# HJakeCunningham/ASVGP

Hardware: AMD Instinct MI355X
Metric: Mpoints/s per ELBO+grad step, N=10M 1D Matern-3/2 M=2048 (higher is better)
Workload: dtype f64

## Files before the change

### asvgp_amd/csrc/bcr_mfma.hpp

```cpp
#pragma once
#include "bcr.hpp"
#include "prior_plan.hpp"

namespace asvgp {

constexpr int BM_THREADS = 1024;
constexpr int BM_B = 4;
constexpr int BM_GAT = 0, BM_GBT = 16, BM_DINV = 32, BM_SD = 48, BM_CAT = 64, BM_CBT = 80, BM_W = 96, BM_DG = 100, BM_REC = 104;

__host__ __device__ inline size_t bcr_mfma_ws_doubles(long nb) { return (size_t)nb * BM_REC + 64; }
__host__ __device__ inline size_t bcr_mfma_lds_doubles(long nb) {
  return (size_t)((nb + 1) / 2 + 1) * 32 + (size_t)nb * 4 + 96 + (size_t)(BM_THREADS / 64) * 4 * 40 + (size_t)(nb / 8 + 2) * 52;
}

__device__ __forceinline__ double bm_mfma(double a, double b, double c) { return __builtin_amdgcn_mfma_f64_4x4x4f64(a, b, c, 0, 0, 0); }

__device__ __forceinline__ double bm_chol_linv(const double (&d)[10], int hi, int lo, double& dprod, int& badj) {
  double l00, i0, l10, l20, l30, l11, i1, l21, l31, l22, i2, l32, l33, i3;
  Num<double>::sqrt_inv(d[0], l00, i0);
  badj = !(d[0] > 0.0) ? 1 : 0;
  l10 = d[1] * i0; l20 = d[3] * i0; l30 = d[6] * i0;
  double s = fma(-l10, l10, d[2]);
  badj = (!(s > 0.0) && !badj) ? 2 : badj;
  Num<double>::sqrt_inv(s, l11, i1);
  l21 = fma(-l20, l10, d[4]) * i1;
  l31 = fma(-l30, l10, d[7]) * i1;
  s = fma(-l21, l21, fma(-l20, l20, d[5]));
  badj = (!(s > 0.0) && !badj) ? 3 : badj;
  Num<double>::sqrt_inv(s, l22, i2);
  l32 = fma(-l31, l21, fma(-l30, l20, d[8])) * i2;
  s = fma(-l32, l32, fma(-l31, l31, fma(-l30, l30, d[9])));
  badj = (!(s > 0.0) && !badj) ? 4 : badj;
  Num<double>::sqrt_inv(s, l33, i3);
  dprod = (l00 * l11) * (l22 * l33);
  const double z0 = (lo == 0) ? i0 : 0.0;
  const double z1 = fma(-l10, z0, (lo == 1) ? 1.0 : 0.0) * i1;
  const double z2 = fma(-l21, z1, fma(-l20, z0, (lo == 2) ? 1.0 : 0.0)) * i2;
  const double z3 = fma(-l32, z2, fma(-l31, z1, fma(-l30, z0, (lo == 3) ? 1.0 : 0.0))) * i3;
  return hi == 0 ? z0 : (hi == 1 ? z1 : (hi == 2 ? z2 : z3));
}

template <typename Src> __device__ __forceinline__ auto bm_src_load(const Src& A, int dd, long col, long M, int) -> decltype(A.load_dc(dd, col, M)) {
  return A.load_dc(dd, col, M);
}
template <typename Src> __device__ __forceinline__ double bm_src_load(const Src& A, int dd, long col, long M, long) {
  return A.load((long)dd * M + col, true);
}
struct BmLog {
  double m; int e;
  __device__ __forceinline__ void mul(double p) {
    m *= p;
    const int hi = __double2hiint(m);
    e += ((hi >> 20) & 0x7ff) - 1023;
    m = __hiloint2double((hi & 0x800fffff) | 0x3ff00000, __double2loint(m));
  }
};

__device__ __forceinline__ unsigned long long bm_wave_xor(unsigned long long x) {
#pragma unroll
  for (int off = 32; off > 0; off >>= 1) x ^= (unsigned long long)__shfl_xor((long long)x, off, 64);
  return x;
}
__device__ __forceinline__ void bm_msg_send(double* box, int n, double v, unsigned long long tag, int lane) {
  unsigned long long* b = reinterpret_cast<unsigned long long*>(box);
  const unsigned long long w = lane < n ? (unsigned long long)__double_as_longlong(v) : 0ull;
  const unsigned long long x = bm_wave_xor(w) ^ tag;
  if (lane < n) __hip_atomic_store(b + lane, w, __ATOMIC_RELAXED, __HIP_MEMORY_SCOPE_AGENT);
  if (lane == n) __hip_atomic_store(b + n, x, __ATOMIC_RELAXED, __HIP_MEMORY_SCOPE_AGENT);
}
__device__ __forceinline__ bool bm_msg_recv(const double* box, int n, double& v, unsigned long long tag, int lane, long spin_limit) {
  const unsigned long long* b = reinterpret_cast<const unsigned long long*>(box);
  for (long spins = 0; spins <= spin_limit; ++spins) {
    const unsigned long long w = lane <= n ? __hip_atomic_load(b + lane, __ATOMIC_RELAXED, __HIP_MEMORY_SCOPE_AGENT) : 0ull;
    const unsigned long long x = bm_wave_xor(lane < n ? w : 0ull) ^ tag;
    const unsigned long long chk = (unsigned long long)__shfl((long long)w, n, 64);
    if (x == chk) { v = __longlong_as_double((long long)w); return true; }
    __builtin_amdgcn_s_sleep(1);
  }
  return false;
}

struct BmSplit {
  int half = -1;
  double* xchg = nullptr;
  long spin_limit = 0;
  int* gave_up = nullptr;
  unsigned long long tag = 0;
};
constexpr int BM_XCHG = 96;

template <typename Src>
__device__ __attribute__((always_inline)) void bcr_mfma_solve(Src A, const double* rhs, int M, double* ws, double* lds, double* Sband, double* x,
                                                              double* logdet, int* info, int rhs_stride = 1, double* stamps = nullptr,
                                                              BmSplit sp = BmSplit{}) {
  constexpr int B = BM_B;
  const int tid = threadIdx.x;
  const int lane = tid & 63, wv = __builtin_amdgcn_readfirstlane(tid >> 6);
  const int r = lane >> 4, q = (lane >> 2) & 3, c = lane & 3;
  const int e = r * 4 + c, et = c * 4 + r;
  const int hi = r > c ? r : c, lo = r > c ? c : r;
  const int nb = (M + B - 1) / B;
  const int nslot = (nb + 1) / 2;
  double* Dl = lds;
  double* El = lds + (size_t)(nslot + 1) * 16;
  double* xs = El + (size_t)(nslot + 1) * 16;
  double* red = xs + (size_t)nb * B;
  double* slab = red + 96 + (size_t)(wv * 4 + q) * 40;
  double* Fl = red + 96 + (size_t)(BM_THREADS / 64) * 4 * 40;
  double* Sl = lds;
  int levels = 0;
  while ((1 << levels) < nb) ++levels;
  const bool split = sp.half >= 0;
  const int top = levels - 1, ht = 1 << (top > 0 ? top : 0);
  double s_other = 0.0;
  int bad_other = 0x7fffffff;
  auto level_share = [&](int l, int ne, int& m0, int& ne_h) {
    m0 = 0; ne_h = ne;
    if (!split) return;
    if (l < top) {
      const int mL = ht >> (l + 1);
      if (sp.half == 0) ne_h = ne < mL ? ne : mL;
      else { m0 = mL; ne_h = ne > mL ? ne - mL : 0; }
    } else {
      ne_h = sp.half == 0 ? ne : 0;
    }
  };
  int bad = 0;
  BmLog ld{1.0, 0};
  unsigned long long t_prev = stamps ? __builtin_amdgcn_s_memtime() : 0ull;
  int nst = 0;
  auto stamp = [&]() {
    if (stamps && tid == 0) { const unsigned long long t = __builtin_amdgcn_s_memtime(); stamps[nst++] = (double)(t - t_prev); t_prev = t; }
  };
  auto rec = [&](int node) -> double* { return ws + (size_t)node * BM_REC; };
  auto bandD = [&](int n, int rr, int cc) -> double {
    const int col = n * B + cc, row = n * B + rr;
    const bool pad = row >= M;
    const double v = bm_src_load(A, rr - cc, pad ? 0 : col, (long)M, 0);
    return pad ? ((rr == cc) ? 1.0 : 0.0) : v;
  };
  auto bandE = [&](int n, int rr, int cc) -> double {
    if (rr > cc) return 0.0;
    const int col = n * B + cc, row = (n + 1) * B + rr;
    const bool pad = row >= M;
    const double v = bm_src_load(A, B + rr - cc, pad ? 0 : col, (long)M, 0);
    return pad ? 0.0 : v;
  };
  if ((nb & 1) && tid < 16 && !(split && sp.half == 0)) {
    const int rr = tid >> 2, cc = tid & 3;
    Dl[(size_t)((nb - 1) >> 1) * 16 + tid] = bandD(nb - 1, rr > cc ? rr : cc, rr > cc ? cc : rr);
  }
  if (split && sp.half == 0 && tid < 16) Dl[(size_t)(ht >> 1) * 16 + tid] = 0.0;
  for (int row = tid; row < nb * B; row += BM_THREADS) {
    const bool sep_left = split && sp.half == 0 && row >= ht * B && row < (ht + 1) * B;
    xs[row] = (row < M && !sep_left) ? rhs[(long)row * rhs_stride] : 0.0;
  }
  __syncthreads();
  stamp();

  constexpr int RMAXR = 4;
  for (int l = 0; l < levels; ++l) {
    const int h = 1 << l;
    const int ne = (nb > h) ? (nb - h + 2 * h - 1) / (2 * h) : 0;
    int m0, ne_h;
    level_share(l, ne, m0, ne_h);
    if (split && l == top) {
      if (sp.half == 1) {
        if (wv == 0) {
          const double v = lane < 16 ? Dl[(size_t)(ht >> 1) * 16 + lane] : (lane < 20 ? xs[ht * B + lane - 16] : 0.0);
          bm_msg_send(sp.xchg, 20, v, sp.tag | 1ull, lane);
        }
        const double mine = (r == 0 && c == 0) ? (log(ld.m) + (double)ld.e * 0.6931471805599453094) : 0.0;
        const double tot = wave_sum_dpp(mine);
        int bm = bad ? bad : 0x7fffffff;
#pragma unroll
        for (int off = 32; off > 0; off >>= 1) { const int o = __shfl_xor(bm, off, 64); bm = o < bm ? o : bm; }
        int* sbad = reinterpret_cast<int*>(red + 32);
        if (lane == 0) { red[wv] = tot; sbad[wv] = bm; }
        __syncthreads();
        if (wv == 0) {
          double sv = 0.0;
          int bmin = 0x7fffffff;
          for (int w2 = 0; w2 < BM_THREADS / 64; ++w2) { sv += red[w2]; bmin = sbad[w2] < bmin ? sbad[w2] : bmin; }
          bm_msg_send(sp.xchg + 24, 2, lane == 0 ? sv : (double)bmin, sp.tag | 2ull, lane);
        }
      } else {
        if (wv == 0) {
          double v = 0.0;
          if (!bm_msg_recv(sp.xchg, 20, v, sp.tag | 1ull, lane, sp.spin_limit)) { if (lane == 0) *sp.gave_up = 1; }
          else {
            if (lane < 16) Dl[(size_t)(ht >> 1) * 16 + lane] += v;
            else if (lane < 20) xs[ht * B + lane - 16] += v;
          }
        }
        __syncthreads();
        if (*sp.gave_up) return;
      }
      stamp();
    }
    double updb[RMAXR], ybu[RMAXR];
    int qv = q, ev = e;
    asm volatile("" : "+v"(qv), "+v"(ev));
    double sl[2][3];
    auto slab_loads = [&](int rd0) __attribute__((always_inline)) {
#pragma unroll
      for (int u = 0; u < 2; ++u) {
#pragma unroll
        for (int t3 = 0; t3 < 3; ++t3) {
          sl[u][t3] = 0.0;
          int m = (rd0 + u) * 64 + wv * 4 + qv;
          m = m0 + (m < ne_h ? m : ne_h - 1);
          const int kk = ev + 16 * t3, dd = kk >> 3, col = m * 2 * B + (kk & 7);
          const bool in = kk < 40 && col + dd < M;
          const double v = bm_src_load(A, in ? dd : 0, in ? col : 0, (long)M, 0);
          sl[u][t3] = in ? v : ((dd == 0) ? 1.0 : 0.0);
        }
      }
    };
#pragma unroll
    for (int rd = 0; rd < RMAXR; ++rd) {
      __builtin_amdgcn_sched_barrier(0);
      if (l == 0 && (rd & 1) == 0) slab_loads(rd);
      updb[rd] = 0.0; ybu[rd] = 0.0;
      if (rd * 64 + wv * 4 >= ne_h) continue;
      const int ml = rd * 64 + wv * 4 + q;
      const bool act = ml < ne_h;
      const int i = h + (m0 + (act ? ml : ne_h - 1)) * 2 * h, a = i - h, b = i + h;
      const bool hasb = b < nb;
      const int bsafe = hasb ? b : a;
      double d[10];
      double ea, eb, da;
      if (l == 0) {
#pragma unroll
        for (int t3 = 0; t3 < 3; ++t3) if (e + 16 * t3 < 40) slab[e + 16 * t3] = sl[rd & 1][t3];
        int kk = 0;
#pragma unroll
        for (int rr = 0; rr < 4; ++rr)
#pragma unroll
          for (int cc = 0; cc <= rr; ++cc) d[kk++] = slab[(rr - cc) * 8 + 4 + cc];
        ea = slab[(4 + lo - hi) * 8 + hi];
        ea = (r <= c) ? ea : 0.0;
        eb = slab[(4 + lo - hi) * 8 + 4 + hi];
        eb = (hasb && c <= r) ? eb : 0.0;
        da = slab[(hi - lo) * 8 + lo];
      } else {
        const double* Di = Dl + (size_t)(i >> 1) * 16;
        int kk = 0;
#pragma unroll
        for (int rr = 0; rr < 4; ++rr)
#pragma unroll
          for (int cc = 0; cc <= rr; ++cc) d[kk++] = Di[rr * 4 + cc];
        ea = El[(size_t)(a >> 1) * 16 + e];
        eb = El[(size_t)(i >> 1) * 16 + et];
        eb = hasb ? eb : 0.0;
        da = Dl[(size_t)(a >> 1) * 16 + e];
      }
      double yv = xs[i * B + r], ya = xs[a * B + r];
      yv = (c == 0) ? yv : 0.0;
      ya = (c == 0) ? ya : 0.0;
      (void)bsafe;
      double dprod;
      int badj;
      const double t = bm_chol_linv(d, hi, lo, dprod, badj);
      if (act && badj && !bad) bad = i * B + badj;
      const double linv = (r >= c) ? t : 0.0;
      const double linvT = (c >= r) ? t : 0.0;
      if (act) ld.mul(dprod);
      const double ua = bm_mfma(linvT, ea, 0.0);
      const double ub = bm_mfma(linvT, eb, 0.0);
      const double zz = bm_mfma(linvT, yv, 0.0);
      const double nua = -ua, nub = -ub;
      const double da_new = bm_mfma(nua, ua, da);
      const double e_new = bm_mfma(nub, ua, 0.0);
      const double ya_new = bm_mfma(nua, zz, ya);
      updb[rd] = bm_mfma(ub, ub, 0.0);
      ybu[rd] = bm_mfma(ub, zz, 0.0);
      updb[rd] = act ? updb[rd] : 0.0;
      ybu[rd] = act ? ybu[rd] : 0.0;
      const double gat = bm_mfma(ua, linv, 0.0);
      const double gbt = bm_mfma(ub, linv, 0.0);
      const double dinv = bm_mfma(linv, linv, 0.0);
      const double w = bm_mfma(linv, zz, 0.0);
      if (act) {
        if (l >= 3) {
          double* R = Fl + (size_t)(i >> 3) * 52;
          R[e] = gat; R[16 + e] = gbt; R[32 + e] = dinv;
          if (c == 0) R[48 + r] = w;
        } else {
          double* R = rec(i);
          R[BM_GAT + e] = gat; R[BM_GBT + e] = gbt; R[BM_DINV + e] = dinv;
          if (c == 0) R[BM_W + r] = w;
        }
        Dl[(size_t)(a >> 1) * 16 + e] = da_new;
        El[(size_t)(a >> 1) * 16 + e] = e_new;
        if (c == 0) xs[a * B + r] = ya_new;
      }
    }
    bcr_lds_barrier();
#pragma unroll
    for (int rd = 0; rd < RMAXR; ++rd) {
      if (rd * 64 + wv * 4 >= ne_h) continue;
      const int ml = rd * 64 + wv * 4 + q;
      const int i = h + (m0 + ml) * 2 * h, b = i + h;
      if (ml < ne_h && b < nb) {
        Dl[(size_t)(b >> 1) * 16 + e] -= updb[rd];
        if (c == 0) xs[b * B + r] -= ybu[rd];
      }
    }
    bcr_lds_barrier();
    stamp();
  }
  if (wv == 0 && !(split && sp.half == 1)) {
    const bool act = q == 0;
    double d[10];
    int kk = 0;
#pragma unroll
    for (int rr = 0; rr < 4; ++rr)
#pragma unroll
      for (int cc = 0; cc <= rr; ++cc) { const double v = Dl[rr * 4 + cc]; d[kk++] = act ? v : ((rr == cc) ? 1.0 : 0.0); }
    const double yv = (act && c == 0) ? xs[r] : 0.0;
    double dprod;
    int badj;
    const double t = bm_chol_linv(d, hi, lo, dprod, badj);
    if (act && badj && !bad) bad = badj;
    const double linv = (r >= c) ? t : 0.0, linvT = (c >= r) ? t : 0.0;
    if (act) ld.mul(dprod);
    const double s00 = bm_mfma(linv, linv, 0.0);
    const double zz = bm_mfma(linvT, yv, 0.0);
    const double x0 = bm_mfma(linv, zz, 0.0);
    if (act) {
      rec(0)[BM_SD + e] = s00;
      Sl[e] = s00;
      if (r >= c && r < M) Sband[(long)(r - c) * M + c] = s00;
      if (c == 0) xs[r] = x0;
    }
  }
  __syncthreads();
  stamp();
  unsigned long long lw = 0ull;
  for (int l = levels - 1; l >= 0; --l) {
    const int h = 1 << l;
    const int ne = (nb > h) ? (nb - h + 2 * h - 1) / (2 * h) : 0;
    int m0, ne_h;
    level_share(l, ne, m0, ne_h);
    if (split && sp.half == 0 && wv == BM_THREADS / 64 - 1) {
      if (l == top - 1 && lane <= 2)
        lw = __hip_atomic_load(reinterpret_cast<const unsigned long long*>(sp.xchg + 24) + lane, __ATOMIC_RELAXED, __HIP_MEMORY_SCOPE_AGENT);
      if (l == 2) {
        const unsigned long long x = bm_wave_xor(lane < 2 ? lw : 0ull) ^ (sp.tag | 2ull);
        const unsigned long long chk = (unsigned long long)__shfl((long long)lw, 2, 64);
        double v = __longlong_as_double((long long)lw);
        bool ok = x == chk;
        if (!ok) ok = bm_msg_recv(sp.xchg + 24, 2, v, sp.tag | 2ull, lane, sp.spin_limit);
        if (!ok) { if (lane == 0) *sp.gave_up = 1; }
        else if (lane < 2) red[48 + lane] = v;
      }
    }
#pragma unroll
    for (int rd = 0; rd < RMAXR; ++rd) {
      __builtin_amdgcn_sched_barrier(0);
      if (rd * 64 + wv * 4 >= ne_h) continue;
      const int ml = rd * 64 + wv * 4 + q;
      const bool act = ml < ne_h;
      const int i = h + (m0 + (act ? ml : ne_h - 1)) * 2 * h, a = i - h, b = i + h;
      const bool hasb = b < nb;
      const int bs = hasb ? b : a;
      const bool e_is_a = ((a / (2 * h)) & 1) != 0;
      double gat, gbt, dinv, w, saa, sbb, sba, sab;
      if (l >= 3) {
        const double* R = Fl + (size_t)(i >> 3) * 52;
        gat = R[e]; gbt = R[16 + e]; dinv = R[32 + e]; w = R[48 + r];
      } else {
        const double* R = rec(i);
        gat = R[BM_GAT + e]; gbt = R[BM_GBT + e]; dinv = R[BM_DINV + e]; w = R[BM_W + r];
      }
      if (l >= 1) {
        const double* Ra = Sl + (size_t)(a >> 2) * 48;
        const double* Rb = Sl + (size_t)(bs >> 2) * 48;
        saa = Ra[e];
        sbb = Rb[e];
        sba = e_is_a ? Ra[32 + e] : Rb[16 + et];
        sab = e_is_a ? Ra[32 + et] : Rb[16 + e];
      } else {
        const double* Ra = rec(a);
        const double* Rb = rec(bs);
        saa = Ra[BM_SD + e];
        sbb = Rb[BM_SD + e];
        sba = e_is_a ? Ra[BM_CBT + e] : Rb[BM_CAT + et];
        sab = e_is_a ? Ra[BM_CBT + et] : Rb[BM_CAT + e];
      }
      sbb = hasb ? sbb : 0.0; sba = hasb ? sba : 0.0; sab = hasb ? sab : 0.0;
      double xa = xs[a * B + r], xb = xs[bs * B + r];
      xa = (c == 0) ? xa : 0.0;
      xb = (hasb && c == 0) ? xb : 0.0;
      w = (c == 0) ? w : 0.0;
      double ncat = bm_mfma(saa, gat, 0.0);
      ncat = bm_mfma(sba, gbt, ncat);
      double ncbt = bm_mfma(sab, gat, 0.0);
      ncbt = bm_mfma(sbb, gbt, ncbt);
      double sii = bm_mfma(ncat, gat, dinv);
      sii = bm_mfma(ncbt, gbt, sii);
      double gx = bm_mfma(gat, xa, 0.0);
      gx = bm_mfma(gbt, xb, gx);
      if (act) {
        if (c == 0) xs[i * B + r] = w - gx;
        if (l >= 2) {
          double* Rw = Sl + (size_t)(i >> 2) * 48;
          Rw[e] = sii; Rw[16 + e] = -ncat; Rw[32 + e] = -ncbt;
        }
        if (l > 0) {
          double* Rw = rec(i);
          Rw[BM_SD + e] = sii; Rw[BM_CAT + e] = -ncat; Rw[BM_CBT + e] = -ncbt;
        }
        if (r >= c && i * B + r < M) Sband[(long)(r - c) * M + i * B + c] = sii;
        if (l == 0) {
          if (c <= r && i * B + c < M) Sband[(long)(B + c - r) * M + a * B + r] = -ncat;
          if (hasb && r <= c && b * B + r < M) Sband[(long)(B + r - c) * M + i * B + c] = -ncbt;
        }
      }
    }
    if (l == 1) __syncthreads(); else bcr_lds_barrier();
    if (split && l == top) {
      double* Rs = Sl + (size_t)(ht >> 2) * 48;
      if (sp.half == 0) {
        if (wv == 0) bm_msg_send(sp.xchg + 32, 52, lane < 48 ? Rs[lane < 48 ? lane : 0] : (lane < 52 ? xs[ht * B + lane - 48] : 0.0), sp.tag | 3ull, lane);
      } else {
        if (wv == 0) {
          double v = 0.0;
          if (!bm_msg_recv(sp.xchg + 32, 52, v, sp.tag | 3ull, lane, sp.spin_limit)) { if (lane == 0) *sp.gave_up = 1; }
          else if (lane < 48) {
            Rs[lane] = v;
            rec(ht)[BM_SD + lane] = v;
            if (lane < 16) {
              const int rr = lane >> 2, cc = lane & 3;
              if (rr >= cc && ht * B + rr < M) Sband[(long)(rr - cc) * M + ht * B + cc] = v;
            }
          } else if (lane < 52) {
            xs[ht * B + lane - 48] = v;
          }
        }
        __syncthreads();
        if (*sp.gave_up) return;
      }
    }
    stamp();
  }
  if (!(split && sp.half == 0))
    for (int col = M - B + tid; col < M; col += BM_THREADS)
      if (col >= 0)
#pragma unroll
        for (int dd = 1; dd <= B; ++dd)
          if (col + dd >= M) Sband[(long)dd * M + col] = 0.0;
  {
    const int row0 = (split && sp.half == 1) ? (ht + 1) * B : 0, row1 = (split && sp.half == 0) ? (ht + 1) * B : M;
    for (int row = row0 + tid; row < row1 && row < M; row += BM_THREADS) x[(long)row * rhs_stride] = xs[row];
  }
  if (!(split && sp.half == 1)) {
    const double mine = (r == 0 && c == 0) ? (log(ld.m) + (double)ld.e * 0.6931471805599453094) : 0.0;
    const double tot = wave_sum_dpp(mine);
    int bm = bad ? bad : 0x7fffffff;
#pragma unroll
    for (int off = 32; off > 0; off >>= 1) { const int o = __shfl_xor(bm, off, 64); bm = o < bm ? o : bm; }
    int* sbad = reinterpret_cast<int*>(red + 32);
    if (lane == 0) { red[wv] = tot; sbad[wv] = bm; }
    __syncthreads();
    if (split && tid == 0) { s_other = red[48]; bad_other = (int)red[49]; }
    if (tid == 0) {
      double s = 0.0;
      int bmin = 0x7fffffff;
      for (int w2 = 0; w2 < BM_THREADS / 64; ++w2) { s += red[w2]; bmin = sbad[w2] < bmin ? sbad[w2] : bmin; }
      s += s_other;
      bmin = bad_other < bmin ? bad_other : bmin;
      __hip_atomic_store(logdet + 0, 2.0 * s, __ATOMIC_RELAXED, __HIP_MEMORY_SCOPE_AGENT);
      __hip_atomic_store(logdet + 1, 0.0, __ATOMIC_RELAXED, __HIP_MEMORY_SCOPE_AGENT);
      __hip_atomic_store(info, (bmin == 0x7fffffff) ? 0 : bmin, __ATOMIC_RELAXED, __HIP_MEMORY_SCOPE_AGENT);
    }
  }
  stamp();
}


__host__ __device__ inline size_t bcr_mfma_pre_ws_doubles(long nb) { return (size_t)nb * 96 + 64; }
__host__ __device__ inline size_t bcr_mfma_pre_lds_doubles(long nb, int n_rec) {
  return PRIOR_TAB_HEADER + (size_t)2 * n_rec * prior_rec_fields(BM_B) + (size_t)(nb / 4 + 2) * 96 + (size_t)(nb + 1) / 2 + 64;
}

struct BmDual { double v, d; };
__device__ __forceinline__ BmDual bm_dmfma(BmDual x, BmDual y, BmDual c) {
  BmDual r;
  r.v = bm_mfma(x.v, y.v, c.v);
  r.d = bm_mfma(x.d, y.v, c.d);
  r.d = bm_mfma(x.v, y.d, r.d);
  return r;
}

__device__ __attribute__((always_inline)) void bcr_mfma_backward_pre(const double* __restrict__ tab, int n_rec, const int* __restrict__ node_rec, int M,
                                                                      double* ws, double* lds, double* Sv, double* Sd, double* logdet, int* info,
                                                                      unsigned long long* done_flag, unsigned long long seq,
                                                                      const unsigned long long* ready_flag = nullptr, long spin_limit = 0, int* gave_up = nullptr) {
  constexpr int B = BM_B, W = prior_rec_fields(B);
  const int tid = threadIdx.x;
  if (ready_flag) {
    if (tid == 0) {
      long spins = 0;
      while (__hip_atomic_load(ready_flag, __ATOMIC_RELAXED, __HIP_MEMORY_SCOPE_SYSTEM) < seq) {
        __builtin_amdgcn_s_sleep(8);
        if (++spins > spin_limit) { *gave_up = 1; break; }
      }
    }
    __syncthreads();
    if (*gave_up) return;
    __builtin_amdgcn_fence(__ATOMIC_ACQUIRE, "");
  }
  const int lane = tid & 63, wv = __builtin_amdgcn_readfirstlane(tid >> 6);
  const int r = lane >> 4, q = (lane >> 2) & 3, c = lane & 3;
  const int e = r * 4 + c, et = c * 4 + r;
  const int nb = (M + B - 1) / B;
  const int n_tab = PRIOR_TAB_HEADER + 2 * n_rec * W;
  double* tl = lds;
  double* Sl = lds + n_tab;
  int* nrl = reinterpret_cast<int*>(Sl + (size_t)(nb / 4 + 2) * 96);
  {
    const double2* src = reinterpret_cast<const double2*>(tab);
    double2* dst = reinterpret_cast<double2*>(tl);
    for (int i2 = tid; i2 < n_tab / 2; i2 += BM_THREADS) dst[i2] = src[i2];
    for (int i2 = tid; i2 < nb; i2 += BM_THREADS) nrl[i2] = node_rec[i2];
  }
  __syncthreads();
  if (done_flag && tid == 0) __hip_atomic_store(done_flag, seq, __ATOMIC_RELAXED, __HIP_MEMORY_SCOPE_SYSTEM);
  const double* tv = tl + PRIOR_TAB_HEADER;
  const double* td = tv + (size_t)n_rec * W;
  int levels = 0;
  while ((1 << levels) < nb) ++levels;
  if (tid < 16) {
    const int r0 = nrl[0];
    const double xv = tv[(size_t)r0 * W + prior_f_UA(B) + tid], xd = td[(size_t)r0 * W + prior_f_UA(B) + tid];
    Sl[tid] = xv; Sl[48 + tid] = xd;
    ws[tid] = xv; ws[48 + tid] = xd;
    const int rr = tid >> 2, cc = tid & 3;
    if (rr >= cc && rr < M) { Sv[(long)(rr - cc) * M + cc] = xv; Sd[(long)(rr - cc) * M + cc] = xd; }
  }
// ... 79 lines not shown
```

### asvgp_amd/csrc/elbo.hip

```cpp
#include <stdlib.h>
#include <time.h>
#include <string.h>

#include "bcr_pre.hpp"
#include "bcr_mfma.hpp"
#include "handle.hpp"

namespace asvgp {


struct Ws {
  double *Kuu, *dK, *P, *LK, *dLK, *LP, *SK, *dSK, *SP, *c, *alpha, *logdets, *fin, *bcrK, *bcrP;
};
static size_t bcr_ws_chain(int planes, int k, bool big) {
  long ns = 1024;
  while ((long)planes * 2 * k * k * ns * 8 + 2 * ns * k * 8 + 1024 > 150 * 1024) ns >>= 1;
  if (big) ns *= 2;
  return (size_t)planes * (7 * k * k + k) * 2 * ns + (big ? (size_t)planes * k * k * ns : 0);
}
static size_t bcr_ws_K(int k, long M) {
  size_t a = bcr_ws_chain(2, k, false), b = bcr_ws_chain(2, k, true), c = bcr_pre_ws_doubles(k, (M + k - 1) / k);
  a = a > b ? a : b;
  return (a > c ? a : c) + 64;
}
static size_t bcr_ws_P(int k) { size_t a = bcr_ws_chain(1, k, false), b = bcr_ws_chain(1, k, true); return (a > b ? a : b) + 64; }
static size_t bcr_ws_total(long M, int k) { return bcr_ws_K(k, M) + bcr_ws_P(k); }
static size_t ws_doubles(long M, int k, long D) {
  return (size_t)9 * (k + 1) * M + (size_t)2 * M * D + 64 + 32 + bcr_ws_total(M, k);
}
static Ws carve(void* ws, long M, int k, long D) {
  double* p = static_cast<double*>(ws);
  size_t E = (size_t)(k + 1) * M;
  Ws w;
  w.Kuu = p; p += E; w.dK = p; p += E; w.P = p; p += E; w.LK = p; p += E; w.dLK = p; p += E;
  w.LP = p; p += E; w.SK = p; p += E; w.dSK = p; p += E; w.SP = p; p += E;
  w.c = p; p += (size_t)M * D; w.alpha = p; p += (size_t)M * D;
  w.logdets = p; p += 64;
  w.fin = p; p += 32;
  w.bcrK = p; p += bcr_ws_K(k, M);
  w.bcrP = p;
  return w;
}

template <int K> struct ElboLauncher {
  static int run(Handle* h, const double* stats, const double* S, int kind, double v, double l, double s, long N, long M, long D,
                 double* out, int* info, void* ws, hipStream_t st, int part);
};
template <int K> struct KuuInvLauncher {
  static int run(Handle* h, const double* S, int kind, double v, double l, long M, double* Kuu, double* dK, double* SK, double* dSK,
                 double* logdet2, int* info, void* ws, hipStream_t st);
};
template <int K> struct PostLauncher {
  static int run(Handle* h, const double* stats, const double* S, int kind, double v, double l, double s, long M, long D,
                 double* alpha, double* W, int* info, void* ws, hipStream_t st, double* Pinv = nullptr);
};
static size_t cov_ws_doubles(long M, int k) { return (size_t)4 * (k + 1) * M + (size_t)2 * M + 8; }
template <int K> struct PostCovLauncher {
  static int run(Handle* h, const double* stats, const double* S, int kind, double v, double l, double s, long M, long D,
                 double* alpha, double* W, double* Wd, int* info, void* ws, hipStream_t st);
};

#ifdef ASVGP_ELBO_ONLY_K
struct KuuCoefs2 { double c[ASVGP_MAX_KUU_TERMS]; double dc[ASVGP_MAX_KUU_TERMS]; int n; };

constexpr int KI_DKB = 8;
struct KuuInterior { double k[8]; long lo, hi; double bnd[2 * PRIOR_BND_DIAGS * PRIOR_BND]; double dk[8]; double dkb[2 * 5 * KI_DKB]; int dk_tab; };
struct ThetaBox {
  unsigned long long seq;
  double s, alpha_scale, v, l, N, Nw, cw;
  double k[8], dk[8];
  double bnd[2 * PRIOR_BND_DIAGS * PRIOR_BND];
  double dkb[2 * 5 * KI_DKB];
  double dc[ASVGP_MAX_KUU_TERMS];
};
typedef const __attribute__((address_space(3))) double* lds_cdouble_ptr;
struct BandSumToep {
  const double* A; double inv_s;
  lds_cdouble_ptr kl;
  lds_cdouble_ptr bnd;
  long lo, hi;
  __device__ __forceinline__ double load_dc(int dd, long col, long M) const {
#pragma clang fp contract(off)
    const double t2 = A[(long)dd * M + col] * inv_s;
    const bool left = col < lo, right = col >= hi;
    const long bi = left ? (long)dd * PRIOR_BND + col : (right ? (long)(PRIOR_BND_DIAGS + dd) * PRIOR_BND + (col - hi) : 0);
    const double bv = bnd[bi];
    const double kv = kl[dd];
    return t2 + ((left || right) ? bv : kv);
  }
};

static __global__ void elbo_prepare_kernel(const double* __restrict__ S, KuuCoefs2 cf, long E, const double* __restrict__ A,
                                    double s, double* __restrict__ Kuu, double* __restrict__ dK,
                                    double* __restrict__ P) {
#pragma clang fp contract(off)
  long e = (long)blockIdx.x * blockDim.x + threadIdx.x;
  if (e >= E) return;
  double acc = cf.c[0] * S[e];
  double dacc = cf.dc[0] * S[e];
  for (int t = 1; t < cf.n; ++t) {
    double sv = S[(long)t * E + e];
    acc = acc + cf.c[t] * sv;
    dacc = dacc + cf.dc[t] * sv;
  }
  Kuu[e] = acc;
  if (dK) dK[e] = dacc;
  if (P) P[e] = A[e] / s + acc;
}

template <int K, bool TANGENT, bool RHS>
__global__ __launch_bounds__(64) void elbo_factor_kernel(const double* Kuu, const double* dK, const double* P,
                                                         double* LK, double* dLK, double* LP, const double* b,
                                                         double* c, int M, int* info) {
  if (blockIdx.x == 0) {
    if (TANGENT) cholesky_sweep<Dual, K, false>(BandPtr<Dual>{Kuu, dK}, BandOut<Dual>{LK, dLK}, M, nullptr, nullptr, info);
    else cholesky_sweep<double, K, false>(BandPtr<double>{Kuu, nullptr}, BandOut<double>{LK, nullptr}, M, nullptr, nullptr, info);
  } else {
    cholesky_sweep<double, K, RHS>(BandPtr<double>{P, nullptr}, BandOut<double>{LP, nullptr}, M, b, c, info + 1);
  }
}

template <int K, bool TANGENT, bool RHS>
__global__ __launch_bounds__(64) void elbo_inverse_kernel(const double* LK, const double* dLK, const double* LP,
                                                          double* SK, double* dSK, double* SP, const double* c,
                                                          double* alpha, int M) {
  if (blockIdx.x == 0) {
    if (TANGENT) takahashi_sweep<Dual, K, false>(BandPtr<Dual>{LK, dLK}, BandOut<Dual>{SK, dSK}, M, nullptr, nullptr);
    else takahashi_sweep<double, K, false>(BandPtr<double>{LK, nullptr}, BandOut<double>{SK, nullptr}, M, nullptr, nullptr);
  } else {
    takahashi_sweep<double, K, RHS>(BandPtr<double>{LP, nullptr}, BandOut<double>{SP, nullptr}, M, c, alpha);
  }
}

template <int K>
__global__ __launch_bounds__(64) void elbo_trsv_kernel(const double* L, int M, const double* B, double* X, long D,
                                                       int trans, double scale) {
  const long d = blockIdx.x;
  if (trans) trsv_sweep<K, true>(L, M, B + d, X + d, D);
  else trsv_sweep<K, false>(L, M, B + d, X + d, D);
  (void)scale;
}

template <int K, bool BIG>
__device__ __forceinline__ void more_columns(const double* b, double* x, int D, int M, double* wsP, double* lds, int lds_doubles) {
  if (D <= 1) return;
  __syncthreads();
  const int nb = (M + K - 1) / K;
  int chunk = lds_doubles / (nb * K);
  if (chunk < 1) chunk = 1;
// ... 503 lines not shown
    tot[CC] = tot[BA] / sn;
    const double two_pi = 6.283185307179586476925286766559;
    double elbo = -0.5 * N * log(two_pi * sn);
    elbo -= 0.5 * tot[LOGP];
    elbo += 0.5 * tot[LOGK];
    elbo -= 0.5 * yy / sn;
    elbo += 0.5 * tot[CC];
    elbo -= 0.5 * Nw * v / sn;
    elbo += 0.5 * tot[TRKA] / sn;
    if (th_v.cw != 0.0) elbo += th_v.cw;
    const double d_l = 0.5 * (tot[SKDK] - tot[SPDK] - tot[ADKA] + tot[DTRKA] / sn);
    const double d_v = 0.5 * (-tot[SKK] / v + tot[SPK] / v + tot[AKA] / v + tot[TRKA] / (v * sn)) - 0.5 * Nw / sn;
    const double s2 = sn * sn;
    const double d_s = -0.5 * N / sn + 0.5 * tot[SPA] / s2 + 0.5 * yy / s2 + 0.5 * tot[AAA] / s2 - tot[BA] / s2 + 0.5 * Nw * v / s2 - 0.5 * tot[TRKA] / s2;
    double* out = fin.out;
    out[0] = elbo; out[1] = d_v; out[2] = d_l; out[3] = d_s;
    out[4] = tot[LOGK]; out[5] = tot[LOGP]; out[6] = tot[TRKA]; out[7] = tot[CC];
    if (fin.mirror) {
      double* m = fin.mirror;
      const double mv[10] = {elbo, d_v, d_l, d_s, tot[LOGK], tot[LOGP], tot[TRKA], tot[CC],
                             (double)__hip_atomic_load(info, __ATOMIC_RELAXED, __HIP_MEMORY_SCOPE_AGENT),
                             (double)__hip_atomic_load(info + 1, __ATOMIC_RELAXED, __HIP_MEMORY_SCOPE_AGENT)};
      double sum = (double)fin.mirror_seq;
#pragma unroll
      for (int i = 0; i < 10; ++i) { __hip_atomic_store(m + i, mv[i], __ATOMIC_RELAXED, __HIP_MEMORY_SCOPE_SYSTEM); sum += mv[i]; }
      __hip_atomic_store(m + 11, sum, __ATOMIC_RELAXED, __HIP_MEMORY_SCOPE_SYSTEM);
      __hip_atomic_store(m + 10, (double)fin.mirror_seq, __ATOMIC_RELAXED, __HIP_MEMORY_SCOPE_SYSTEM);
    }
  }
  rstamp(2);
}

static __global__ void scale_sub_kernel(const double* __restrict__ a, const double* __restrict__ b, double* __restrict__ o,
                                 long n) {
  long i = (long)blockIdx.x * blockDim.x + threadIdx.x;
  if (i < n) o[i] = a[i] - b[i];
}
static __global__ void scale_kernel(double* __restrict__ x, double f, long n) {
  long i = (long)blockIdx.x * blockDim.x + threadIdx.x;
  if (i < n) x[i] = x[i] * f;
}

template <int K, bool TANGENT>
static int run_chains(Handle* h, const double* stats, const double* S, int kind, double v, double l, double s, long M, long D,
                      Ws w, int* info, hipStream_t st, bool& use_bcr, int part = 0, bool scale_alpha = true, FusedFin* fin = nullptr) {
  double t_enter = 0.0;
  if (debug_env().host_times) { timespec ts; clock_gettime(CLOCK_MONOTONIC, &ts); t_enter = ts.tv_sec * 1e6 + ts.tv_nsec * 1e-3; }
  KuuCoefs2 cf;
  for (int t = 0; t < ASVGP_MAX_KUU_TERMS; ++t) cf.c[t] = cf.dc[t] = 0.0;
  int rc = asvgp_matern_coeffs(kind, v, l, cf.c, cf.dc, &cf.n);
  if (rc) return rc;
  const long E = (long)(K + 1) * M;
  const double* A = stats;
  const double* b = stats ? stats + E : nullptr;
  const long nb = (M + K - 1) / K;
  const int algo = h->band_algo;
  const bool have_plan = h->plan && prior_plan_M(h->plan) == M && prior_plan_k(h->plan) == K && prior_plan_terms(h->plan) == cf.n;
  if ((algo == 3 || algo == 4) && !have_plan) { set_error("band algorithms 3 and 4 need asvgp_prior_plan_1d for this (M, k, kernel)"); return ASVGP_ERR_BAD_ARG; }
  size_t ldsK = sizeof(double) * (TANGENT ? bcr_lds_doubles<Dual, K, 0>(nb) : bcr_lds_doubles<double, K, 0>(nb));
  size_t ldsP = sizeof(double) * bcr_lds_doubles<double, K, 1>(nb);
  bool planned = have_plan && (algo == 0 || algo == 3 || algo == 4);
  size_t lds_bytes = planned ? ldsP : (ldsK > ldsP ? ldsK : ldsP);
  bool fits = lds_bytes <= 160 * 1024 - 256;
  bool big = false;
  constexpr bool HAS_BIG = (K <= 5);
  if (HAS_BIG && !fits) {
    size_t bK = sizeof(double) * (TANGENT ? bcr_lds_doubles<Dual, K, 0, true>(nb) : bcr_lds_doubles<double, K, 0, true>(nb));
    size_t bP = sizeof(double) * bcr_lds_doubles<double, K, 1, true>(nb);
    size_t bb = planned ? bP : (bK > bP ? bK : bP);
    if (bb <= 160 * 1024 - 256) { big = true; fits = true; lds_bytes = bb; }
  }
  use_bcr = (algo == 2 || algo == 3 || algo == 4 || (algo == 0 && fits));
  planned = planned && use_bcr;
  if (part != 0 && (!use_bcr || planned)) {
    if (part == 1) return ASVGP_OK;
    part = 0;
  }
  if (planned) {
    const int n_rec = prior_plan_nrec(h->plan);
    bool use_mfma = false;
    KuuInterior ki;
    if constexpr (K == BM_B) {
      use_mfma = (algo == 0 || algo == 4) && D == 1 && nb <= 512 && TANGENT && fin != nullptr &&
                 sizeof(double) * bcr_mfma_lds_doubles(nb) <= 160 * 1024 && sizeof(double) * bcr_mfma_pre_lds_doubles(nb, n_rec) <= 160 * 1024;
      if (use_mfma) {
        prior_plan_interior_kuu(h->plan, cf.c, ki.k, &ki.lo, &ki.hi, ki.bnd);
        use_mfma = ki.hi > ki.lo;
        if (use_mfma) {
          double bnd2[2 * PRIOR_BND_DIAGS * PRIOR_BND];
          long lo2 = 0, hi2 = 0;
          prior_plan_interior_kuu(h->plan, cf.dc, ki.dk, &lo2, &hi2, bnd2);
          ki.dk_tab = (ki.lo <= KI_DKB && M - ki.hi <= KI_DKB) ? 1 : 0;
          for (int sd = 0; sd < 2; ++sd)
            for (int d = 0; d <= K; ++d)
              for (int cI = 0; cI < KI_DKB; ++cI)
                ki.dkb[(sd * 5 + d) * KI_DKB + cI] = bnd2[(size_t)(sd * PRIOR_BND_DIAGS + d) * PRIOR_BND + cI];
        }
      }
    }
    if (algo == 4 && !use_mfma) {
      set_error("band algorithm 4 (matrix-core chains) needs k = 4, D = 1, M <= 2048, Toeplitz static bands and the ELBO + gradient entry point");
      return ASVGP_ERR_UNSUPPORTED;
    }
    if (h->ahead_req && !use_mfma) { set_error("launch-ahead exists for the matrix-core launch only (k = 4, D = 1, M <= 2048, planned prior chain)"); return ASVGP_ERR_UNSUPPORTED; }
    if (!use_mfma && !fits) { set_error("BCR needs %zu B of LDS", lds_bytes); return ASVGP_ERR_LDS_CAPACITY; }
    unsigned long long seq = 0;
    int slot = 0;
    double t_acq0 = 0.0, t_acq1 = 0.0;
    if (debug_env().host_times) { timespec ts; clock_gettime(CLOCK_MONOTONIC, &ts); t_acq0 = ts.tv_sec * 1e6 + ts.tv_nsec * 1e-3; }
    double* tab = handle_table_acquire(h, &seq, &slot);
    if (debug_env().host_times) { timespec ts; clock_gettime(CLOCK_MONOTONIC, &ts); t_acq1 = ts.tv_sec * 1e6 + ts.tv_nsec * 1e-3; }
    const bool gpu_fwd = h->prior_forward_gpu;
    const double* tab_k = h->tab_dev + (size_t)slot * h->slot_doubles;
    const unsigned long long* dd_ready = nullptr;
    if (gpu_fwd) {
      double* t = nullptr;
      rc = handle_prior_dd_forward(h, cf.c, cf.dc, slot, st, &t, nullptr, use_mfma ? seq : 0ull, use_mfma ? &dd_ready : nullptr);
      if (rc) return rc;
      tab_k = t;
    }
    size_t lds_pre = sizeof(double) * bcr_pre_lds_doubles(K, n_rec);
    if (lds_pre > lds_bytes) lds_bytes = lds_pre;
    FusedFin ff{};
    if (fin) { ff = *fin; ff.finalize = 1; fin->finalize = -1; }
    ff.n_helpers = (int)((M + 255) / 256 < 6 ? (M + 255) / 256 : 6);
    ff.split = 0; ff.xchg = nullptr;
    ff.assembled = reinterpret_cast<unsigned*>(w.fin + 20);
    ff.debug_no_assembly = debug_env().no_assembly;
    ff.debug_stamps = debug_env().chain_stamps;
    const long spin_limit = debug_env().spin_limit;
    if constexpr (K == BM_B) {
      if (use_mfma) {
        size_t lb = sizeof(double) * bcr_mfma_lds_doubles(nb), lk = sizeof(double) * bcr_mfma_pre_lds_doubles(nb, n_rec);
        if (lk > lb) lb = lk;
        if (sizeof(double) * FIN_LDS_DOUBLES > lb) lb = sizeof(double) * FIN_LDS_DOUBLES;
        auto kern = elbo_chains_mfma_kernel<K>;
        static size_t lds_granted[16] = {0};
        size_t& granted = lds_granted[h->device & 15];
        if (lb > granted) {
          hipError_t e = hipFuncSetAttribute(reinterpret_cast<const void*>(kern), hipFuncAttributeMaxDynamicSharedMemorySize, (int)lb);
          if (e != hipSuccess) { set_error("hipFuncSetAttribute: %s", hipGetErrorString(e)); return ASVGP_ERR_LDS_CAPACITY; }
          granted = lb;
        }
        if (h->mirror_dev) { ff.mirror = h->mirror_dev; ff.mirror_seq = ++h->mirror_seq; h->mirror_pending = ff.mirror_seq; }
        if (nb >= 128 && !debug_env().no_split) {
          ff.split = 1;
          ff.xchg = w.LP;
        }
        ff.n_helpers = 0;
        const bool plan_first = debug_env().plan_first != 0;
        const bool host_times = debug_env().host_times != 0;
        auto now_us = []() { timespec ts; clock_gettime(CLOCK_MONOTONIC, &ts); return ts.tv_sec * 1e6 + ts.tv_nsec * 1e-3; };
        const double t0 = host_times ? now_us() : 0.0;
        if (plan_first && !gpu_fwd) (void)prior_plan_eval(h->plan, cf.c, cf.dc, tab);
        const ThetaBox* box_k = nullptr;
        if (h->ahead_req) {
          if (gpu_fwd || plan_first) { set_error("launch-ahead needs the host forward pass (asvgp_set_prior_forward(h, 0))"); return ASVGP_ERR_UNSUPPORTED; }
          static_assert(sizeof(ThetaBox) <= BOX_BYTES, "theta box");
          if (!h->box_host) {
            if (hipHostMalloc(&h->box_host, BOX_BYTES * TAB_SLOTS, hipHostMallocMapped | hipHostMallocPortable | hipHostMallocCoherent) != hipSuccess ||
                hipHostGetDevicePointer(&h->box_dev, h->box_host, 0) != hipSuccess) {
              if (h->box_host) { (void)hipHostFree(h->box_host); h->box_host = nullptr; }
              set_error("launch-ahead: pinned allocation failed: %s", hipGetErrorString(hipGetLastError()));
              return ASVGP_ERR_HIP;
            }
            memset(h->box_host, 0, BOX_BYTES * TAB_SLOTS);
          }
// ... 589 lines not shown
```

Baseline: 131,200.

## Factor 4x4 diagonal blocks once per lane before MFMA rounds in wide levels

In the MFMA block cyclic-reduction solver, wide levels now get a separate pre-pass. Each lane factors one whole 4x4 diagonal block and writes its L^-1 entries to LDS, instead of all 16 lanes of a block redundantly running the same Cholesky and picking out one entry. The slab area becomes one shared double-buffered region that also holds the L^-1 records, rounds are processed in pairs, and the log-det accumulation is restricted to one lane per block. This removes redundant scalar Cholesky work but adds extra LDS barriers and round trips per level. The LDS budget check now also counts the kernel's static LDS.

```diff
diff --git a/asvgp_amd/csrc/bcr_mfma.hpp b/asvgp_amd/csrc/bcr_mfma.hpp
--- a/asvgp_amd/csrc/bcr_mfma.hpp
+++ b/asvgp_amd/csrc/bcr_mfma.hpp
@@ -9,35 +9,50 @@
 constexpr int BM_GAT = 0, BM_GBT = 16, BM_DINV = 32, BM_SD = 48, BM_CAT = 64, BM_CBT = 80, BM_W = 96, BM_DG = 100, BM_REC = 104;
 
 __host__ __device__ inline size_t bcr_mfma_ws_doubles(long nb) { return (size_t)nb * BM_REC + 64; }
+constexpr int BM_SLAB = 40;
+constexpr int BM_SLABS = 2 * 64 * BM_SLAB;
+constexpr int BM_LREC = 260;
+static_assert(10 * BM_LREC <= BM_SLABS, "the L^-1 records of a wide level live in the slab area");
 __host__ __device__ inline size_t bcr_mfma_lds_doubles(long nb) {
-  return (size_t)((nb + 1) / 2 + 1) * 32 + (size_t)nb * 4 + 96 + (size_t)(BM_THREADS / 64) * 4 * 40 + (size_t)(nb / 8 + 2) * 52;
+  return (size_t)((nb + 1) / 2 + 1) * 32 + (size_t)nb * 4 + 96 + (size_t)BM_SLABS + (size_t)(nb / 8 + 2) * 52;
 }
 
 __device__ __forceinline__ double bm_mfma(double a, double b, double c) { return __builtin_amdgcn_mfma_f64_4x4x4f64(a, b, c, 0, 0, 0); }
 
+struct BmChol {
+  double l10, l20, l30, l21, l31, l32, i0, i1, i2, i3;
+  __device__ __forceinline__ void factor(const double (&d)[10], double& dprod, int& badj) {
+    double l00, l11, l22, l33;
+    Num<double>::sqrt_inv(d[0], l00, i0);
+    badj = !(d[0] > 0.0) ? 1 : 0;
+    l10 = d[1] * i0; l20 = d[3] * i0; l30 = d[6] * i0;
+    double s = fma(-l10, l10, d[2]);
+    badj = (!(s > 0.0) && !badj) ? 2 : badj;
+    Num<double>::sqrt_inv(s, l11, i1);
+    l21 = fma(-l20, l10, d[4]) * i1;
+    l31 = fma(-l30, l10, d[7]) * i1;
+    s = fma(-l21, l21, fma(-l20, l20, d[5]));
+    badj = (!(s > 0.0) && !badj) ? 3 : badj;
+    Num<double>::sqrt_inv(s, l22, i2);
+    l32 = fma(-l31, l21, fma(-l30, l20, d[8])) * i2;
+    s = fma(-l32, l32, fma(-l31, l31, fma(-l30, l30, d[9])));
+    badj = (!(s > 0.0) && !badj) ? 4 : badj;
+    Num<double>::sqrt_inv(s, l33, i3);
+    dprod = (l00 * l11) * (l22 * l33);
+  }
+  __device__ __forceinline__ void column(int lo, double (&z)[4]) const {
+    z[0] = (lo == 0) ? i0 : 0.0;
+    z[1] = fma(-l10, z[0], (lo == 1) ? 1.0 : 0.0) * i1;
+    z[2] = fma(-l21, z[1], fma(-l20, z[0], (lo == 2) ? 1.0 : 0.0)) * i2;
+    z[3] = fma(-l32, z[2], fma(-l31, z[1], fma(-l30, z[0], (lo == 3) ? 1.0 : 0.0))) * i3;
+  }
+};
 __device__ __forceinline__ double bm_chol_linv(const double (&d)[10], int hi, int lo, double& dprod, int& badj) {
-  double l00, i0, l10, l20, l30, l11, i1, l21, l31, l22, i2, l32, l33, i3;
-  Num<double>::sqrt_inv(d[0], l00, i0);
-  badj = !(d[0] > 0.0) ? 1 : 0;
-  l10 = d[1] * i0; l20 = d[3] * i0; l30 = d[6] * i0;
-  double s = fma(-l10, l10, d[2]);
-  badj = (!(s > 0.0) && !badj) ? 2 : badj;
-  Num<double>::sqrt_inv(s, l11, i1);
-  l21 = fma(-l20, l10, d[4]) * i1;
-  l31 = fma(-l30, l10, d[7]) * i1;
-  s = fma(-l21, l21, fma(-l20, l20, d[5]));
-  badj = (!(s > 0.0) && !badj) ? 3 : badj;
-  Num<double>::sqrt_inv(s, l22, i2);
-  l32 = fma(-l31, l21, fma(-l30, l20, d[8])) * i2;
-  s = fma(-l32, l32, fma(-l31, l31, fma(-l30, l30, d[9])));
-  badj = (!(s > 0.0) && !badj) ? 4 : badj;
-  Num<double>::sqrt_inv(s, l33, i3);
-  dprod = (l00 * l11) * (l22 * l33);
-  const double z0 = (lo == 0) ? i0 : 0.0;
-  const double z1 = fma(-l10, z0, (lo == 1) ? 1.0 : 0.0) * i1;
-  const double z2 = fma(-l21, z1, fma(-l20, z0, (lo == 2) ? 1.0 : 0.0)) * i2;
-  const double z3 = fma(-l32, z2, fma(-l31, z1, fma(-l30, z0, (lo == 3) ? 1.0 : 0.0))) * i3;
-  return hi == 0 ? z0 : (hi == 1 ? z1 : (hi == 2 ? z2 : z3));
+  BmChol ch;
+  ch.factor(d, dprod, badj);
+  double z[4];
+  ch.column(lo, z);
+  return hi == 0 ? z[0] : (hi == 1 ? z[1] : (hi == 2 ? z[2] : z[3]));
 }
 
 template <typename Src> __device__ __forceinline__ auto bm_src_load(const Src& A, int dd, long col, long M, int) -> decltype(A.load_dc(dd, col, M)) {
@@ -105,8 +120,8 @@
   double* El = lds + (size_t)(nslot + 1) * 16;
   double* xs = El + (size_t)(nslot + 1) * 16;
   double* red = xs + (size_t)nb * B;
-  double* slab = red + 96 + (size_t)(wv * 4 + q) * 40;
-  double* Fl = red + 96 + (size_t)(BM_THREADS / 64) * 4 * 40;
+  double* slabs = red + 96;
+  double* Fl = slabs + BM_SLABS;
   double* Sl = lds;
   int levels = 0;
   while ((1 << levels) < nb) ++levels;
@@ -170,7 +185,7 @@
           const double v = lane < 16 ? Dl[(size_t)(ht >> 1) * 16 + lane] : (lane < 20 ? xs[ht * B + lane - 16] : 0.0);
           bm_msg_send(sp.xchg, 20, v, sp.tag | 1ull, lane);
         }
-        const double mine = (r == 0 && c == 0) ? (log(ld.m) + (double)ld.e * 0.6931471805599453094) : 0.0;
+        const double mine = log(ld.m) + (double)ld.e * 0.6931471805599453094;
         const double tot = wave_sum_dpp(mine);
         int bm = bad ? bad : 0x7fffffff;
 #pragma unroll
@@ -199,8 +214,8 @@
       stamp();
     }
     double updb[RMAXR], ybu[RMAXR];
-    int qv = q, ev = e;
-    asm volatile("" : "+v"(qv), "+v"(ev));
+    int qv = q, ev = e, lv = lane;
+    asm volatile("" : "+v"(qv), "+v"(ev), "+v"(lv));
     double sl[2][3];
     auto slab_loads = [&](int rd0) __attribute__((always_inline)) {
 #pragma unroll
@@ -217,39 +232,84 @@
         }
       }
     };
-#pragma unroll
-    for (int rd = 0; rd < RMAXR; ++rd) {
-      __builtin_amdgcn_sched_barrier(0);
-      if (l == 0 && (rd & 1) == 0) slab_loads(rd);
+    auto slab_of = [&](int rd, int slot) -> double* { return slabs + (size_t)((rd & 1) * 64 + slot) * BM_SLAB; };
+    auto stage = [&](int rd) __attribute__((always_inline)) {
+      if (rd * 64 + wv * 4 >= ne_h) return;
+      double* slab = slab_of(rd, wv * 4 + qv);
+#pragma unroll
+      for (int t3 = 0; t3 < 3; ++t3) if (e + 16 * t3 < BM_SLAB) slab[e + 16 * t3] = sl[rd & 1][t3];
+    };
+    const bool wide = ne_h > 16;
+    auto factor = [&](int rd) __attribute__((always_inline)) {
+      const int ml = rd * 64 + lv;
+      if (rd * 64 + (lv & ~3) >= ne_h) return;
+      const bool act = ml < ne_h;
+      const int i = h + (m0 + (act ? ml : ne_h - 1)) * 2 * h;
+      double d[10];
+      double* slab = slab_of(rd, lv);
+      const double* Di = Dl + (size_t)(i >> 1) * 16;
+      int kk = 0;
+#pragma unroll
+      for (int rr = 0; rr < 4; ++rr)
+#pragma unroll
+        for (int cc = 0; cc <= rr; ++cc, ++kk) {
+          if (l == 0) d[kk] = slab[(rr - cc) * 8 + 4 + cc];
+          else d[kk] = Di[rr * 4 + cc];
+        }
+      BmChol ch;
+      double dprod;
+      int badj;
+      ch.factor(d, dprod, badj);
+      if (act && badj && !bad) bad = i * B + badj;
+      if (act) ld.mul(dprod);
+#pragma unroll
+      for (int cc = 0; cc < 4; ++cc) {
+        double z[4];
+        ch.column(cc, z);
+#pragma unroll
+        for (int rr = cc; rr < 4; ++rr) {
+          if (l == 0) slab[(rr - cc) * 8 + 4 + cc] = z[rr];
+          else slabs[(rr * (rr + 1) / 2 + cc) * BM_LREC + ml] = z[rr];
+        }
+      }
+    };
+    auto round = [&](int rd, bool pre) __attribute__((always_inline)) {
       updb[rd] = 0.0; ybu[rd] = 0.0;
-      if (rd * 64 + wv * 4 >= ne_h) continue;
+      if (rd * 64 + wv * 4 >= ne_h) return;
       const int ml = rd * 64 + wv * 4 + q;
       const bool act = ml < ne_h;
       const int i = h + (m0 + (act ? ml : ne_h - 1)) * 2 * h, a = i - h, b = i + h;
       const bool hasb = b < nb;
       const int bsafe = hasb ? b : a;
       double d[10];
-      double ea, eb, da;
+      double ea, eb, da, t;
       if (l == 0) {
-#pragma unroll
-        for (int t3 = 0; t3 < 3; ++t3) if (e + 16 * t3 < 40) slab[e + 16 * t3] = sl[rd & 1][t3];
-        int kk = 0;
-#pragma unroll
-        for (int rr = 0; rr < 4; ++rr)
-#pragma unroll
-          for (int cc = 0; cc <= rr; ++cc) d[kk++] = slab[(rr - cc) * 8 + 4 + cc];
+        const double* slab = slab_of(rd, wv * 4 + qv);
+        if (pre) {
+          t = slab[(hi - lo) * 8 + 4 + lo];
+        } else {
+          int kk = 0;
+#pragma unroll
+          for (int rr = 0; rr < 4; ++rr)
+#pragma unroll
+            for (int cc = 0; cc <= rr; ++cc) d[kk++] = slab[(rr - cc) * 8 + 4 + cc];
+        }
         ea = slab[(4 + lo - hi) * 8 + hi];
         ea = (r <= c) ? ea : 0.0;
         eb = slab[(4 + lo - hi) * 8 + 4 + hi];
         eb = (hasb && c <= r) ? eb : 0.0;
         da = slab[(hi - lo) * 8 + lo];
       } else {
-        const double* Di = Dl + (size_t)(i >> 1) * 16;
-        int kk = 0;
-#pragma unroll
-        for (int rr = 0; rr < 4; ++rr)
-#pragma unroll
-          for (int cc = 0; cc <= rr; ++cc) d[kk++] = Di[rr * 4 + cc];
+        if (pre) {
+          t = slabs[(hi * (hi + 1) / 2 + lo) * BM_LREC + rd * 64 + wv * 4 + qv];
+        } else {
+          const double* Di = Dl + (size_t)(i >> 1) * 16;
+          int kk = 0;
+#pragma unroll
+          for (int rr = 0; rr < 4; ++rr)
+#pragma unroll
+            for (int cc = 0; cc <= rr; ++cc) d[kk++] = Di[rr * 4 + cc];
+        }
         ea = El[(size_t)(a >> 1) * 16 + e];
         eb = El[(size_t)(i >> 1) * 16 + et];
         eb = hasb ? eb : 0.0;
@@ -259,13 +319,15 @@
       yv = (c == 0) ? yv : 0.0;
       ya = (c == 0) ? ya : 0.0;
       (void)bsafe;
-      double dprod;
-      int badj;
-      const double t = bm_chol_linv(d, hi, lo, dprod, badj);
-      if (act && badj && !bad) bad = i * B + badj;
+      if (!pre) {
+        double dprod;
+        int badj;
+        t = bm_chol_linv(d, hi, lo, dprod, badj);
+        if (act && badj && !bad) bad = i * B + badj;
+        if (act && e == 0) ld.mul(dprod);
+      }
       const double linv = (r >= c) ? t : 0.0;
       const double linvT = (c >= r) ? t : 0.0;
-      if (act) ld.mul(dprod);
       const double ua = bm_mfma(linvT, ea, 0.0);
       const double ub = bm_mfma(linvT, eb, 0.0);
       const double zz = bm_mfma(linvT, yv, 0.0);
@@ -286,15 +348,31 @@
           double* R = Fl + (size_t)(i >> 3) * 52;
           R[e] = gat; R[16 + e] = gbt; R[32 + e] = dinv;
           if (c == 0) R[48 + r] = w;
+          asm volatile("" ::: "memory");
         } else {
           double* R = rec(i);
           R[BM_GAT + e] = gat; R[BM_GBT + e] = gbt; R[BM_DINV + e] = dinv;
           if (c == 0) R[BM_W + r] = w;
+          asm volatile("" ::: "memory");
         }
         Dl[(size_t)(a >> 1) * 16 + e] = da_new;
         El[(size_t)(a >> 1) * 16 + e] = e_new;
         if (c == 0) xs[a * B + r] = ya_new;
       }
+    };
+#pragma unroll
+    for (int rp = 0; rp < RMAXR; rp += 2) {
+      __builtin_amdgcn_sched_barrier(0);
+      const bool any = rp * 64 < ne_h;
+      if (l == 0 && any) { slab_loads(rp); stage(rp); stage(rp + 1); }
+      if (wide && (l == 0 ? any : rp == 0)) {
+        if (l == 0) bcr_lds_barrier();
+        if (wv < (l == 0 ? 2 : RMAXR)) factor(l == 0 ? rp + wv : wv);
+        bcr_lds_barrier();
+      }
+      round(rp, wide);
+      __builtin_amdgcn_sched_barrier(0);
+      round(rp + 1, wide);
     }
     bcr_lds_barrier();
 #pragma unroll
@@ -324,7 +402,7 @@
     const double t = bm_chol_linv(d, hi, lo, dprod, badj);
     if (act && badj && !bad) bad = badj;
     const double linv = (r >= c) ? t : 0.0, linvT = (c >= r) ? t : 0.0;
-    if (act) ld.mul(dprod);
+    if (act && e == 0) ld.mul(dprod);
     const double s00 = bm_mfma(linv, linv, 0.0);
     const double zz = bm_mfma(linvT, yv, 0.0);
     const double x0 = bm_mfma(linv, zz, 0.0);
@@ -370,9 +448,11 @@
       if (l >= 3) {
         const double* R = Fl + (size_t)(i >> 3) * 52;
         gat = R[e]; gbt = R[16 + e]; dinv = R[32 + e]; w = R[48 + r];
+        asm volatile("" ::: "memory");
       } else {
         const double* R = rec(i);
         gat = R[BM_GAT + e]; gbt = R[BM_GBT + e]; dinv = R[BM_DINV + e]; w = R[BM_W + r];
+        asm volatile("" ::: "memory");
       }
       if (l >= 1) {
         const double* Ra = Sl + (size_t)(a >> 2) * 48;
@@ -381,6 +461,7 @@
         sbb = Rb[e];
         sba = e_is_a ? Ra[32 + e] : Rb[16 + et];
         sab = e_is_a ? Ra[32 + et] : Rb[16 + e];
+        asm volatile("" ::: "memory");
       } else {
         const double* Ra = rec(a);
         const double* Rb = rec(bs);
@@ -388,6 +469,7 @@
         sbb = Rb[BM_SD + e];
         sba = e_is_a ? Ra[BM_CBT + e] : Rb[BM_CAT + et];
         sab = e_is_a ? Ra[BM_CBT + et] : Rb[BM_CAT + e];
+        asm volatile("" ::: "memory");
       }
       sbb = hasb ? sbb : 0.0; sba = hasb ? sba : 0.0; sab = hasb ? sab : 0.0;
       double xa = xs[a * B + r], xb = xs[bs * B + r];
@@ -456,7 +538,7 @@
     for (int row = row0 + tid; row < row1 && row < M; row += BM_THREADS) x[(long)row * rhs_stride] = xs[row];
   }
   if (!(split && sp.half == 1)) {
-    const double mine = (r == 0 && c == 0) ? (log(ld.m) + (double)ld.e * 0.6931471805599453094) : 0.0;
+    const double mine = log(ld.m) + (double)ld.e * 0.6931471805599453094;
     const double tot = wave_sum_dpp(mine);
     int bm = bad ? bad : 0x7fffffff;
 #pragma unroll
diff --git a/asvgp_amd/csrc/elbo.hip b/asvgp_amd/csrc/elbo.hip
--- a/asvgp_amd/csrc/elbo.hip
+++ b/asvgp_amd/csrc/elbo.hip
@@ -65,6 +65,7 @@
 
 constexpr int KI_DKB = 8;
 struct KuuInterior { double k[8]; long lo, hi; double bnd[2 * PRIOR_BND_DIAGS * PRIOR_BND]; double dk[8]; double dkb[2 * 5 * KI_DKB]; int dk_tab; };
+constexpr size_t ELBO_MFMA_STATIC_LDS = sizeof(double) * (16 + 2 * PRIOR_BND_DIAGS * PRIOR_BND + 2 * 5 * KI_DKB + 4) + 2 * sizeof(int);
 struct ThetaBox {
   unsigned long long seq;
   double s, alpha_scale, v, l, N, Nw, cw;
@@ -734,7 +735,8 @@
     KuuInterior ki;
     if constexpr (K == BM_B) {
       use_mfma = (algo == 0 || algo == 4) && D == 1 && nb <= 512 && TANGENT && fin != nullptr &&
-                 sizeof(double) * bcr_mfma_lds_doubles(nb) <= 160 * 1024 && sizeof(double) * bcr_mfma_pre_lds_doubles(nb, n_rec) <= 160 * 1024;
+                 sizeof(double) * bcr_mfma_lds_doubles(nb) + ELBO_MFMA_STATIC_LDS <= 160 * 1024 &&
+                 sizeof(double) * bcr_mfma_pre_lds_doubles(nb, n_rec) + ELBO_MFMA_STATIC_LDS <= 160 * 1024;
       if (use_mfma) {
         prior_plan_interior_kuu(h->plan, cf.c, ki.k, &ki.lo, &ki.hi, ki.bnd);
         use_mfma = ki.hi > ki.lo;
```

New measurement: 133,800, median of 4. No clear change (+2.0%).
